# SparklingH/BloomScene

Measured on AMD Instinct MI355X. Metric: Msplats/s fwd+bwd @1M Gaussians 1920x1080 SH3; fraction of HBM roofline, higher is better.
Workload: dtype f32; 1 GPU; c3: 1000000 Gaussians, SH deg 3, 1920x1080, fwd+bwd colour+depth targets, synthetic scene A seed 0; gaussians=1000000, width=1920, height=1080, sh_degree=3, num_rendered=4386625, visible=1000000, parallelism=view-parallel x1, exact_exp=0, strict_gradients=0, prewarm_steps=292

## Files before the change

bloomscene_amd/csrc/api.hip:

```cpp
#include "../../include/bloomscene_rast.h"
#include "common.h"
#include "errors.h"
#include "host_state.h"
#include "launch.h"
#include "profiler.h"
#include "scratch.h"

#include <cstring>

using namespace bsr;

static constexpr unsigned BSR_KNOWN_FLAGS = BSR_FLAG_EXACT_EXP | BSR_FLAG_EXACT_GRAD | BSR_FLAG_NO_READBACK | BSR_FLAG_TEST_MASK;

static bool is_capturing(hipStream_t s)
{
	hipStreamCaptureStatus cs = hipStreamCaptureStatusNone;
	if (hipStreamIsCapturing(s, &cs) != hipSuccess) { (void)hipGetLastError(); cs = hipStreamCaptureStatusNone; }
	return cs != hipStreamCaptureStatusNone;
}

static int check_common(int P, int width, int height, const float* means3D, const float* scales, const float* rotations,
                        const float* cov3D_precomp, const float* viewmatrix, const float* projmatrix)
{
	if (P < 0 || width <= 0 || height <= 0) return fail("invalid sizes: P=%d width=%d height=%d", P, width, height);
// ... 139 lines not shown
	if (P_rows > 0x7fffffffu) return fail("too many (view, Gaussian) pairs for one call");

	char* geom_p = geometryBuffer(geometry_user, GeomState::bytes(P_rows));
	char* img_p = imageBuffer(image_user, ImgState::bytes(N, (size_t)T));
	if (!geom_p || !img_p) return fail("scratch allocation callback returned null");
	ForwardCall c = {s, flags, debug, no_readback, V, P, width, height, gx, gy, T, n_wg, P_rows,
	                 GeomState::carve(geom_p, P_rows), ImgState::carve(img_p, N, (size_t)T),
	                 binningBuffer, binning_user, background, out_color, out_depth, 0};
	const GeomState& geom = c.geom;
	const ImgState& img = c.img;

	if (prefiltered) HIP_TRY(hipMemsetAsync(img.flags, 0, sizeof(int), s));

	{
		PreArgs a;
		memset(&a, 0, sizeof(a));
		a.P = P; a.D = D; a.M = M;
		a.means3D = means3D; a.scales = scales; a.scale_modifier = scale_modifier; a.rotations = rotations;
		a.opacities = opacities; a.shs = shs; a.cov3D_precomp = cov3D_precomp; a.colors_precomp = colors_precomp;
		a.viewmatrix = viewmatrix; a.projmatrix = projmatrix; a.cam_pos = cam_pos;
		a.W = width; a.H = height; a.tan_fovx = tan_fovx; a.tan_fovy = tan_fovy;
		a.focal_y = height / (2.0f * tan_fovy);
		a.focal_x = width / (2.0f * tan_fovx);
		a.gx = gx; a.gy = gy; a.prefiltered = prefiltered; a.radii = radii; a.geom = geom;
		a.flags = img.flags;
		a.n_views = V;
		if (V > 1)
			HIP_TRY(hipMemsetAsync(geom.hist1, 0, BSR_RADIX_BINS_ * hist1_columns((size_t)n_wg) * sizeof(uint32_t), s));
		{
			StageTimer t("preprocess", s);
			launch_preprocess(a, false, s);
		}
		STAGE_CHECK("preprocess", debug, s);
	}
	SyncCache* sc = sync_cache();
	if (!sc) return 1;
	const bool capturing = no_readback && is_capturing(s);
	{
		StageTimer t("scan_wg", s);
		launch_scans(n_wg, geom.wg_kept, geom.wg_area, img.flags, geom.hist1, capturing ? nullptr : sc->pinned_dev, s);
	}
	STAGE_CHECK("scan_wg", debug, s);

	const CallShape shape{P, width, height, V};
	if (no_readback) {
		if (!capturing) {
			HIP_TRY(hipEventRecord(sc->deferred, s));
// ... 289 lines not shown

	if (R > 0) {
		{
			StageTimer t("render_bwd", s);
			RenderBwdArgs w;
			w.gx = gx; w.gy = gy; w.W = width; w.H = height;
			w.tile_range = img.tile_range; w.point_list = bin.point_list; w.rec = geom.rec; w.wg_base = geom.wg_kept;
			w.bg = background; w.final_T = img.final_T; w.n_contrib = img.n_contrib; w.dL_dpix = dL_dpix;
			w.out_depth = out_depth; w.dL_depths = out_depth ? dL_depths : nullptr;
			w.masks_flag = img.flags + 6; w.slab = slab;
			w.strict = (flags & BSR_FLAG_EXACT_GRAD) != 0; w.capacity = R;
			launch_render_bwd(w, s);
		}
		STAGE_CHECK("render_bwd", debug, s);
	}
	BwdArgs a;
	memset(&a, 0, sizeof(a));
	a.P = P; a.D = D; a.M = M;
	a.means3D = means3D; a.radii = radii; a.shs = shs; a.scales = scales; a.rotations = rotations;
	a.scale_modifier = scale_modifier; a.cov3D_precomp = cov3D_precomp; a.viewmatrix = viewmatrix;
	a.projmatrix = projmatrix; a.campos = campos; a.tan_fovx = tan_fovx; a.tan_fovy = tan_fovy;
	a.focal_y = height / (2.0f * tan_fovy);
	a.focal_x = width / (2.0f * tan_fovx);
	a.geom = geom;
	a.slab = slab; a.depth_grad = out_depth != nullptr;
	a.kept_ptr = img.flags + 2; a.capacity = R;
	a.dL_dmean2D = dL_dmean2D; a.dL_dconic = dL_dconic; a.dL_dopacity = dL_dopacity; a.dL_dcolor = dL_dcolor;
	a.dL_dmean3D = dL_dmean3D; a.dL_dcov3D = dL_dcov3D; a.dL_dsh = dL_dsh; a.dL_dscale = dL_dscale; a.dL_drot = dL_drot;
	{
		StageTimer t("preprocess_bwd", s);
		launch_preprocess_bwd(a, s);
	}
	STAGE_CHECK("preprocess_bwd", debug, s);
	return 0;
}

int bsr_backward(int P, int D, int M, int R, const float* background, int width, int height, const float* means3D,
                 const float* shs, const float* colors_precomp, const float* scales, float scale_modifier,
                 const float* rotations, const float* cov3D_precomp, const float* viewmatrix, const float* projmatrix,
                 const float* campos, float tan_fovx, float tan_fovy, const int* radii, char* geom_buffer,
                 char* binning_buffer, char* image_buffer, const float* dL_dpix, const float* dL_depths,
                 float* dL_dmean2D, float* dL_dconic, float* dL_dopacity, float* dL_dcolor, float* dL_dmean3D,
                 float* dL_dcov3D, float* dL_dsh, float* dL_dscale, float* dL_drot, int debug, void* stream)
{
	(void)dL_depths;
	return bsr_backward_ex(P, D, M, R, background, width, height, means3D, shs, colors_precomp, scales, scale_modifier,
	                       rotations, cov3D_precomp, viewmatrix, projmatrix, campos, tan_fovx, tan_fovy, radii, geom_buffer,
// ... 22 lines not shown
```

bloomscene_amd/csrc/common.h:

```cpp
#pragma once
#include <hip/hip_runtime.h>
#include <stdint.h>

#define BSR_TILE 16
#define BSR_BLOCK 256
#define BSR_NEAR 0.2f
#define BSR_PACK_MAX_SRC 8

namespace bsr {

struct Carver;
#define BSR_REC 4
struct GeomState {
	float4* rec;
	uint32_t* inst_offset;
	uint32_t* wg_kept;
	uint32_t* wg_area;
	uint32_t* hist1;
	uint64_t* kept_mask;
	ushort4* rect;
	uint8_t* clamped;
	float* depth;
	static GeomState layout(Carver& c, size_t P);
	static size_t bytes(size_t P);
	static GeomState carve(char* p, size_t P);
};
struct BinElem {
	uint32_t x;
	uint32_t y;
	uint32_t z;
};
typedef float bsr_f32x4 __attribute__((ext_vector_type(4)));
typedef float bsr_f32x2 __attribute__((ext_vector_type(2)));
typedef bsr_f32x4 bsr_f32x4_a4 __attribute__((aligned(4)));
typedef bsr_f32x2 bsr_f32x2_a4 __attribute__((aligned(4)));
__host__ __device__ __forceinline__ constexpr int slab_row_floats(bool depth_grad) { return depth_grad ? 10 : 9; }
#define BSR_SLAB_ROW_BYTES 40
#define BSR_SLAB_TAIL_BYTES 16
typedef uint32_t bsr_u32x3 __attribute__((ext_vector_type(3)));
typedef bsr_u32x3 bsr_u32x3_a4 __attribute__((aligned(4)));
__device__ __forceinline__ BinElem load_elem(const BinElem* p)
{
	const bsr_u32x3 v = *reinterpret_cast<const bsr_u32x3_a4*>(p);
	return BinElem{v.x, v.y, v.z};
}
__device__ __forceinline__ void store_elem(BinElem* p, const BinElem e)
{
	*reinterpret_cast<bsr_u32x3_a4*>(p) = bsr_u32x3{e.x, e.y, e.z};
}
// ... 44 lines not shown
	static size_t bytes(size_t N, size_t T);
	static ImgState carve(char* p, size_t N, size_t T);
};

struct PreArgs {
	int P, D, M;
	const float* means3D;
	const float* scales;
	float scale_modifier;
	const float* rotations;
	const float* opacities;
	const float* shs;
	const float* cov3D_precomp;
	const float* colors_precomp;
	const float* viewmatrix;
	const float* projmatrix;
	const float* cam_pos;
	int W, H;
	float tan_fovx, tan_fovy, focal_x, focal_y;
	int gx, gy;
	int prefiltered;
	int* radii;
	int n_views;
	GeomState geom;
	int* flags;
};

struct BwdArgs {
	int P, D, M;
	const float* means3D;
	const int* radii;
	const float* shs;
	const float* scales;
	const float* rotations;
	float scale_modifier;
	const float* cov3D_precomp;
	const float* viewmatrix;
	const float* projmatrix;
	const float* campos;
	float tan_fovx, tan_fovy, focal_x, focal_y;
	GeomState geom;
	const float4* slab;
	int depth_grad;
	const int* kept_ptr;
	int capacity;
	float* dL_dmean2D;
	float* dL_dconic;
	float* dL_dopacity;
	float* dL_dcolor;
	float* dL_dmean3D;
	float* dL_dcov3D;
	float* dL_dsh;
	float* dL_dscale;
	float* dL_drot;
};

int fail(const char* fmt, ...);

int read_u32_blocking(const uint32_t* dev, uint32_t* out, hipStream_t s);

static inline size_t align_up(size_t x, size_t a) { return (x + a - 1) & ~(a - 1); }

__device__ __forceinline__ float bsr_expf(float x)
{
	if (x != x) return x;
	if (x < -104.0f) return 0.0f;
	if (x > 88.72284f) return __builtin_inff();
	const float k = __builtin_rintf(x * 1.44269504088896341f);
	float r = __builtin_fmaf(-k, 0.693359375f, x);
	r = __builtin_fmaf(-k, -2.12194440e-4f, r);
	float p = 1.0f / 5040.0f;
	p = __builtin_fmaf(p, r, 1.0f / 720.0f);
	p = __builtin_fmaf(p, r, 1.0f / 120.0f);
	p = __builtin_fmaf(p, r, 1.0f / 24.0f);
	p = __builtin_fmaf(p, r, 1.0f / 6.0f);
	p = __builtin_fmaf(p, r, 0.5f);
	p = __builtin_fmaf(p, r, 1.0f);
// ... 125 lines not shown
```

bloomscene_amd/csrc/preprocess.hip:

```cpp
#include "common.h"
#include "sh.h"
#include "tile_common.h"
#include "launch.h"

namespace bsr {

struct Cov2DTerms {
	float t0[3], t1[3];
	float tx, ty, tz;
	float xmul, ymul;
};

__device__ __forceinline__ void cov2d_terms(const float3 mean, float focal_x, float focal_y, float tan_fovx,
                                            float tan_fovy, const float* __restrict__ vm, Cov2DTerms& o)
{
	float tx = vm[0] * mean.x + vm[4] * mean.y + vm[8] * mean.z + vm[12];
	float ty = vm[1] * mean.x + vm[5] * mean.y + vm[9] * mean.z + vm[13];
	const float tz = vm[2] * mean.x + vm[6] * mean.y + vm[10] * mean.z + vm[14];
	const float limx = 1.3f * tan_fovx;
	const float limy = 1.3f * tan_fovy;
	const float txtz = tx / tz;
	const float tytz = ty / tz;
	tx = fminf(limx, fmaxf(-limx, txtz)) * tz;
	ty = fminf(limy, fmaxf(-limy, tytz)) * tz;
// ... 18 lines not shown
	const float A10 = t.t0[0] * c[1] + t.t0[1] * c[3] + t.t0[2] * c[4];
	const float A20 = t.t0[0] * c[2] + t.t0[1] * c[4] + t.t0[2] * c[5];
	const float A01 = t.t1[0] * c[0] + t.t1[1] * c[1] + t.t1[2] * c[2];
	const float A11 = t.t1[0] * c[1] + t.t1[1] * c[3] + t.t1[2] * c[4];
	const float A21 = t.t1[0] * c[2] + t.t1[1] * c[4] + t.t1[2] * c[5];
	a = A00 * t.t0[0] + A10 * t.t0[1] + A20 * t.t0[2];
	b = A01 * t.t0[0] + A11 * t.t0[1] + A21 * t.t0[2];
	cc = A01 * t.t1[0] + A11 * t.t1[1] + A21 * t.t1[2];
	a += 0.3f;
	cc += 0.3f;
}

__device__ __forceinline__ float ndc2pix(float v, int S) { return (float)(((v + 1.0) * S - 1.0) * 0.5); }

__device__ __forceinline__ void get_rect(float px, float py, int max_radius, int gx, int gy, int* rmin, int* rmax)
{
	rmin[0] = min(gx, max(0, (int)((px - max_radius) / BSR_TILE)));
	rmin[1] = min(gy, max(0, (int)((py - max_radius) / BSR_TILE)));
	rmax[0] = min(gx, max(0, (int)((px + max_radius + BSR_TILE - 1) / BSR_TILE)));
	rmax[1] = min(gy, max(0, (int)((py + max_radius + BSR_TILE - 1) / BSR_TILE)));
}


template <bool FILTER_ONLY, int COLOR = 0>
__global__ void __launch_bounds__(256) k_preprocess(const PreArgs a)
{
	const int idx = blockIdx.x * 256 + threadIdx.x;
	const bool in_range = idx < a.P;
	if (FILTER_ONLY && !in_range) return;
	const int view = (int)blockIdx.y;
	const int wg = view * (int)gridDim.x + (int)blockIdx.x;
	const int id = wg * 256 + (int)threadIdx.x;
	const int ty_off = view * a.gy;

	__shared__ uint32_t s_hist[256];
	if (!FILTER_ONLY) {
		s_hist[threadIdx.x] = 0;
		__syncthreads();
	}

	int radius_out = 0;
	ushort4 rect_out = make_ushort4(0, 0, 0, 0);
	uint64_t kept_mask = 0;
	float4 rq0 = make_float4(0.f, 0.f, 0.f, 0.f), rq1 = rq0, rq2 = rq0;

	const int ld = in_range ? idx : 0;
	float3 p = make_float3(a.means3D[3 * ld], a.means3D[3 * ld + 1], a.means3D[3 * ld + 2]);
	const float* vm = a.viewmatrix + 16 * view;
	const float* pm = a.projmatrix + 16 * view;
	float pvz = vm[2] * p.x + vm[6] * p.y + vm[10] * p.z + vm[14];
	const bool alive = in_range && !(pvz <= BSR_NEAR);
	if (in_range && !alive && a.prefiltered) a.flags[0] = 1;

	bool vis = false;
	float cov3D[6] = {0.f, 0.f, 0.f, 0.f, 0.f, 0.f};
	float conic_a = 0.f, conic_b = 0.f, conic_c = 0.f, pix_x = 0.f, pix_y = 0.f;
	int rmin[2] = {0, 0}, rmax[2] = {0, 0};
	if (alive) {
		const float hx = pm[0] * p.x + pm[4] * p.y + pm[8] * p.z + pm[12];
		const float hy = pm[1] * p.x + pm[5] * p.y + pm[9] * p.z + pm[13];
		const float hw = pm[3] * p.x + pm[7] * p.y + pm[11] * p.z + pm[15];
		const float p_w = 1.0f / (hw + 0.0000001f);
		const float projx = hx * p_w, projy = hy * p_w;

		if (a.cov3D_precomp != nullptr) {
#pragma unroll
			for (int k = 0; k < 6; k++) cov3D[k] = a.cov3D_precomp[(size_t)idx * 6 + k];
// ... 65 lines not shown
			if (vis) {
				li = (int)s_pack[0][t];
				p = make_float3(__uint_as_float(s_pack[1][t]), __uint_as_float(s_pack[2][t]), __uint_as_float(s_pack[3][t]));
#pragma unroll
				for (int k = 0; k < 6; k++) cov3D[k] = __uint_as_float(s_pack[4 + k][t]);
				conic_a = __uint_as_float(s_pack[10][t]); conic_b = __uint_as_float(s_pack[11][t]); conic_c = __uint_as_float(s_pack[12][t]);
				radius_out = (int)s_pack[13][t];
				pix_x = __uint_as_float(s_pack[14][t]); pix_y = __uint_as_float(s_pack[15][t]);
				rmin[0] = (int)s_pack[16][t]; rmin[1] = (int)s_pack[17][t];
				rmax[0] = (int)s_pack[18][t]; rmax[1] = (int)s_pack[19][t];
				pvz = __uint_as_float(s_pack[20][t]);
			}
		}
	}
	const int gi = (int)blockIdx.x * 256 + li;
	const int gid = wg * 256 + li;

	if (vis) {
		rect_out = make_ushort4((unsigned short)rmin[0], (unsigned short)(rmin[1] + ty_off),
		                        (unsigned short)rmax[0], (unsigned short)(rmax[1] + ty_off));
		float rgb[3];
		uint8_t clamp_bits = 0;
		if (COLOR == 1) {
			sh3_to_rgb_stream(p, a.cam_pos + 3 * view, a.shs + (size_t)gi * 48, rgb, clamp_bits);
		} else if (COLOR == 0 && a.colors_precomp == nullptr) {
			sh_to_rgb(a.D, a.M, p, a.cam_pos + 3 * view, a.shs + (size_t)gi * a.M * 3, rgb, clamp_bits);
		} else {
			rgb[0] = a.colors_precomp[3 * gi];
			rgb[1] = a.colors_precomp[3 * gi + 1];
			rgb[2] = a.colors_precomp[3 * gi + 2];
		}
		const float opacity = a.opacities[gi];
		const float power_cut = -logf(255.0f * opacity) - 1.0e-3f;
		rq0 = make_float4(pix_x, pix_y, -0.5f * conic_a, -conic_b);
		rq1 = make_float4(-0.5f * conic_c, power_cut, opacity, pvz);
		a.geom.clamped[gid] = clamp_bits;
		const uint32_t area = (uint32_t)(rmax[0] - rmin[0]) * (uint32_t)(rmax[1] - rmin[1]);
		const bool pd = (conic_a > 0.0f) && (conic_c > 0.0f) && (conic_a * conic_c - conic_b * conic_b > 0.0f);
		const float rb_c = -conic_b / conic_c, rb_a = -conic_b / conic_a;
		if (area <= 64u) {
			int x0 = rmin[0], x1 = rmax[0], y0 = rmin[1], y1 = rmax[1];
			const float tq = -(power_cut - (1.0e-3f + 1.0e-4f * fabsf(power_cut)));
			const float cdet = conic_a * conic_c - conic_b * conic_b;
			if (pd) {
				if (tq < 0.0f) {
					x1 = x0;
				} else {
					const float hx = sqrtf(2.0f * tq * conic_c / cdet) * 1.0001f + 0.01f;
					const float hy = sqrtf(2.0f * tq * conic_a / cdet) * 1.0001f + 0.01f;
// ... 43 lines not shown
			const int per = ((int)(gridDim.x * gridDim.y) + 7) >> 3;
			if (a.n_views <= 1 || s_hist[threadIdx.x] != 0u)
				a.geom.hist1[(size_t)threadIdx.x * (8 * per) + hist1_column(wg, per)] = s_hist[threadIdx.x];
		}
		if (threadIdx.x == 0) {
			a.geom.wg_kept[wg] = w0 + w1 + w2 + w3;
			a.geom.wg_area[wg] = s_area[0] + s_area[1] + s_area[2] + s_area[3];
		}
		if (vis) {
			const uint32_t off = (wave > 0 ? w0 : 0u) + (wave > 1 ? w1 : 0u) + (wave > 2 ? w2 : 0u) + incl - n_inst;
			a.geom.rect[gid] = rect_out;
			a.geom.depth[gid] = rq1.w;
			a.geom.inst_offset[gid] = off;
			a.geom.kept_mask[gid] = kept_mask;
			{
				float4* rec = a.geom.rec + (size_t)gid * BSR_REC;
				rec[0] = rq0;
				rec[1] = rq1;
				rec[2] = rq2;
				rec[3] = make_float4(
				    __uint_as_float(off), __uint_as_float((uint32_t)rect_out.x | ((uint32_t)rect_out.y << 16)),
				    __uint_as_float((uint32_t)(rect_out.z - rect_out.x) | ((uint32_t)(rect_out.w - rect_out.y) << 16)),
				    __uint_as_float((uint32_t)kept_mask));
			}
		}
	}
}

__global__ void __launch_bounds__(256) k_mark_visible(int P, const float* __restrict__ means3D,
                                                      const float* __restrict__ vm, uint8_t* __restrict__ present)
{
	const int idx = blockIdx.x * 256 + threadIdx.x;
	if (idx >= P) return;
	const float pvz = vm[2] * means3D[3 * idx] + vm[6] * means3D[3 * idx + 1] + vm[10] * means3D[3 * idx + 2] + vm[14];
	present[idx] = !(pvz <= BSR_NEAR);
}

struct FilterWaveLds {
	float g[9][64];
	uint32_t q[128];
	uint32_t seen[2][64];
};

__device__ __forceinline__ void filter_wave_sync()
{
	__builtin_amdgcn_fence(__ATOMIC_RELEASE, "wavefront");
// ... 166 lines not shown
}

void launch_visible_filter_views(int P, int V, const float* means3D, const float* scales, float scale_modifier,
                                 const float* rotations, const float* cov3D_precomp, const float* viewmatrices,
                                 const float* projmatrices, int W, int H, float tan_fovx, float tan_fovy, int* radii,
                                 const int* group_of_view, int n_groups, uint8_t* group_mask, uint32_t* wg_counts,
                                 uint32_t* group_counts, hipStream_t s)
{
	const int n_wg = (P + 255) / 256;
	hipLaunchKernelGGL(k_visible_filter_views, dim3(n_wg), dim3(256), 0, s, P, V, means3D, scales,
	                   scale_modifier, rotations, cov3D_precomp, viewmatrices, projmatrices, W, H,
	                   W / (2.0f * tan_fovx), H / (2.0f * tan_fovy), tan_fovx, tan_fovy, (W + BSR_TILE - 1) / BSR_TILE,
	                   (H + BSR_TILE - 1) / BSR_TILE, radii, group_of_view, n_groups, group_mask,
	                   group_counts != nullptr ? wg_counts : nullptr);
	if (group_counts != nullptr && n_groups > 0)
		hipLaunchKernelGGL(k_sum_group_counts, dim3(n_groups), dim3(256), 0, s, n_wg, wg_counts, group_counts);
}

void launch_preprocess(const PreArgs& a, bool filter_only, hipStream_t s)
{
	const int blocks = (a.P + 255) / 256;
	if (filter_only)
		hipLaunchKernelGGL((k_preprocess<true, 0>), dim3(blocks), dim3(256), 0, s, a);
	else if (a.colors_precomp == nullptr && a.D == 3 && a.M == 16)
		hipLaunchKernelGGL((k_preprocess<false, 1>), dim3(blocks, a.n_views > 1 ? a.n_views : 1), dim3(256), 0, s, a);
	else if (a.colors_precomp != nullptr)
		hipLaunchKernelGGL((k_preprocess<false, 2>), dim3(blocks, a.n_views > 1 ? a.n_views : 1), dim3(256), 0, s, a);
	else
		hipLaunchKernelGGL((k_preprocess<false, 0>), dim3(blocks, a.n_views > 1 ? a.n_views : 1), dim3(256), 0, s, a);
}

void launch_mark_visible(int P, const float* means3D, const float* vm, uint8_t* present, hipStream_t s)
{
	hipLaunchKernelGGL(k_mark_visible, dim3((P + 255) / 256), dim3(256), 0, s, P, means3D, vm, present);
}

}
```

bloomscene_amd/csrc/preprocess_bwd.hip:

```cpp
#include "common.h"
#include "sh.h"
#include "launch.h"

namespace bsr {


template <int N>
__device__ __forceinline__ void store_sh_grad(float* __restrict__ dst, int M, const float* v)
{
	const int total = M * 3;
	if ((M & 3) == 0) {
		float4* d4 = reinterpret_cast<float4*>(dst);
		constexpr int NV = (N + 3) / 4;
#pragma unroll
		for (int i = 0; i < NV; i++) {
			float4 o;
			o.x = (i * 4 + 0 < N) ? v[i * 4 + 0] : 0.f;
			o.y = (i * 4 + 1 < N) ? v[i * 4 + 1] : 0.f;
			o.z = (i * 4 + 2 < N) ? v[i * 4 + 2] : 0.f;
			o.w = (i * 4 + 3 < N) ? v[i * 4 + 3] : 0.f;
			if (i * 4 < total) d4[i] = o;
		}
		for (int i = NV; i < (total >> 2); i++) d4[i] = make_float4(0.f, 0.f, 0.f, 0.f);
	} else {
#pragma unroll
		for (int i = 0; i < N; i++)
			if (i < total) dst[i] = v[i];
		for (int i = N; i < total; i++) dst[i] = 0.f;
	}
}

__device__ __forceinline__ void zero_sh_grad(float* __restrict__ dst, int M)
{
	const int total = M * 3;
	if ((M & 3) == 0) {
		float4* d4 = reinterpret_cast<float4*>(dst);
		for (int i = 0; i < (total >> 2); i++) d4[i] = make_float4(0.f, 0.f, 0.f, 0.f);
	} else {
		for (int i = 0; i < total; i++) dst[i] = 0.f;
	}
}

template <int DEG>
__device__ __forceinline__ void sh_bwd_deg(const BwdArgs& a, int idx, const float3 m, const float* dcolor, float* dmean)
{
	constexpr int NC = (DEG + 1) * (DEG + 1);
	const float ox = m.x - a.campos[0], oy = m.y - a.campos[1], oz = m.z - a.campos[2];
	const float len = sqrtf((ox * ox + oy * oy) + oz * oz);
	const float x = ox / len, y = oy / len, z = oz / len;
	const uint8_t cl = a.geom.clamped[idx];
	float dL_dRGB[3] = {dcolor[0], dcolor[1], dcolor[2]};
	dL_dRGB[0] *= (cl & 1) ? 0.f : 1.f;
	dL_dRGB[1] *= (cl & 2) ? 0.f : 1.f;
	dL_dRGB[2] *= (cl & 4) ? 0.f : 1.f;
	{
		float dsh[NC * 3];
		sh_coef_grad<DEG>(x, y, z, dL_dRGB, dsh);
		store_sh_grad<NC * 3>(a.dL_dsh + (size_t)idx * a.M * 3, a.M, dsh);
	}
	__builtin_amdgcn_sched_barrier(0);
	float dL_ddir[3];
	{
		float c[NC * 3];
		load_sh<NC>(a.shs + (size_t)idx * a.M * 3, a.M, c);
		sh_dir_grad<DEG>(c, x, y, z, dL_dRGB, dL_ddir);
	}
	const float sum2 = ox * ox + oy * oy + oz * oz;
	const float invsum32 = 1.0f / sqrtf(sum2 * sum2 * sum2);
	dmean[0] += ((+sum2 - ox * ox) * dL_ddir[0] - oy * ox * dL_ddir[1] - oz * ox * dL_ddir[2]) * invsum32;
	dmean[1] += (-ox * oy * dL_ddir[0] + (sum2 - oy * oy) * dL_ddir[1] - oz * oy * dL_ddir[2]) * invsum32;
	dmean[2] += (-ox * oz * dL_ddir[0] - oy * oz * dL_ddir[1] + (sum2 - oz * oz) * dL_ddir[2]) * invsum32;
}

template <int DEG, int ROW_F4>
__device__ __forceinline__ void sh_bwd_coop_half(const BwdArgs& a, int idx, bool visible, const float3 m, const float* dcolor,
                                                 float* dmean, ShTile<ROW_F4, 32>& tile, int lane, int g0, int n_valid)
{
	constexpr int NC = (DEG + 1) * (DEG + 1);
	constexpr int N = NC * 3;
	constexpr int STRIDE = ShTile<ROW_F4, 32>::STRIDE;
	const float ox = m.x - a.campos[0], oy = m.y - a.campos[1], oz = m.z - a.campos[2];
	const float len = sqrtf((ox * ox + oy * oy) + oz * oz);
	const float x = visible ? ox / len : 0.f, y = visible ? oy / len : 0.f, z = visible ? oz / len : 0.f;
	const uint8_t cl = visible ? a.geom.clamped[idx] : (uint8_t)7;
	float dL_dRGB[3] = {0.f, 0.f, 0.f};
	if (visible) {
		dL_dRGB[0] = dcolor[0] * ((cl & 1) ? 0.f : 1.f);
		dL_dRGB[1] = dcolor[1] * ((cl & 2) ? 0.f : 1.f);
		dL_dRGB[2] = dcolor[2] * ((cl & 4) ? 0.f : 1.f);
	}
	const int half = lane >> 5;
	float4* const row = &tile.rows[(lane & 31) * STRIDE];
	{
		float b[NC];
		sh_coef_basis<DEG>(x, y, z, b);
#pragma unroll
		for (int h = 0; h < 2; h++) {
			if (half == h) {
#pragma unroll
				for (int i = 0; i < ROW_F4; i++) {
					float4 o;
					o.x = (i * 4 + 0 < N) ? b[(i * 4 + 0 < N) ? (i * 4 + 0) / 3 : 0] * dL_dRGB[(i * 4 + 0) % 3] : 0.f;
					o.y = (i * 4 + 1 < N) ? b[(i * 4 + 1 < N) ? (i * 4 + 1) / 3 : 0] * dL_dRGB[(i * 4 + 1) % 3] : 0.f;
					o.z = (i * 4 + 2 < N) ? b[(i * 4 + 2 < N) ? (i * 4 + 2) / 3 : 0] * dL_dRGB[(i * 4 + 2) % 3] : 0.f;
					o.w = (i * 4 + 3 < N) ? b[(i * 4 + 3 < N) ? (i * 4 + 3) / 3 : 0] * dL_dRGB[(i * 4 + 3) % 3] : 0.f;
					row[i] = o;
				}
			}
			__builtin_amdgcn_fence(__ATOMIC_RELEASE, "wavefront");
			__builtin_amdgcn_wave_barrier();
			__builtin_amdgcn_fence(__ATOMIC_ACQUIRE, "wavefront");
			sh_tile_store<ROW_F4, 32>(tile, a.dL_dsh, g0 + 32 * h, min(32, max(0, n_valid - 32 * h)), lane);
			__builtin_amdgcn_fence(__ATOMIC_RELEASE, "wavefront");
			__builtin_amdgcn_wave_barrier();
			__builtin_amdgcn_fence(__ATOMIC_ACQUIRE, "wavefront");
		}
	}
	const uint64_t vis_mask = __ballot(visible);
	if (vis_mask == 0ull) return;
	float dL_ddir[3] = {0.f, 0.f, 0.f};
#pragma unroll
	for (int h = 0; h < 2; h++) {
		if (((vis_mask >> (32 * h)) & 0xffffffffull) == 0ull) continue;
		sh_tile_load<ROW_F4, 32>(tile, a.shs, g0 + 32 * h, min(32, max(0, n_valid - 32 * h)), lane);
		__builtin_amdgcn_fence(__ATOMIC_RELEASE, "wavefront");
		__builtin_amdgcn_wave_barrier();
		__builtin_amdgcn_fence(__ATOMIC_ACQUIRE, "wavefront");
		if (visible && half == h) {
			const float* const c = reinterpret_cast<const float*>(row);
			float dx0, dy0, dz0, dx1, dy1, dz1, dx2, dy2, dz2;
			sh_dir_grad_channel<DEG, 0>(c, x, y, z, dx0, dy0, dz0);
			__builtin_amdgcn_sched_barrier(0);
			sh_dir_grad_channel<DEG, 1>(c, x, y, z, dx1, dy1, dz1);
			__builtin_amdgcn_sched_barrier(0);
			sh_dir_grad_channel<DEG, 2>(c, x, y, z, dx2, dy2, dz2);
			dL_ddir[0] = (dx0 * dL_dRGB[0] + dx1 * dL_dRGB[1]) + dx2 * dL_dRGB[2];
			dL_ddir[1] = (dy0 * dL_dRGB[0] + dy1 * dL_dRGB[1]) + dy2 * dL_dRGB[2];
			dL_ddir[2] = (dz0 * dL_dRGB[0] + dz1 * dL_dRGB[1]) + dz2 * dL_dRGB[2];
		}
		__builtin_amdgcn_fence(__ATOMIC_RELEASE, "wavefront");
		__builtin_amdgcn_wave_barrier();
		__builtin_amdgcn_fence(__ATOMIC_ACQUIRE, "wavefront");
	}
	if (visible) {
		const float sum2 = ox * ox + oy * oy + oz * oz;
		const float invsum32 = 1.0f / sqrtf(sum2 * sum2 * sum2);
		dmean[0] += ((+sum2 - ox * ox) * dL_ddir[0] - oy * ox * dL_ddir[1] - oz * ox * dL_ddir[2]) * invsum32;
		dmean[1] += (-ox * oy * dL_ddir[0] + (sum2 - oy * oy) * dL_ddir[1] - oz * oy * dL_ddir[2]) * invsum32;
		dmean[2] += (-ox * oz * dL_ddir[0] - oy * oz * dL_ddir[1] + (sum2 - oz * oz) * dL_ddir[2]) * invsum32;
	}
}

template <int ROW_F4>
__global__ void __launch_bounds__(256, (ROW_F4 == 12 ? 6 : 4)) k_preprocess_bwd(const BwdArgs a)
{
	const int idx = blockIdx.x * 256 + threadIdx.x;
	const bool in_range = idx < a.P;
	const bool overflow = __builtin_amdgcn_readfirstlane(*a.kept_ptr) > a.capacity;
	const ushort4 rc = (in_range && !overflow) ? a.geom.rect[idx] : make_ushort4(0, 0, 0, 0);
	const bool visible = in_range && !overflow && (a.radii ? (a.radii[idx] > 0) : (rc.z > rc.x && rc.w > rc.y));

	constexpr int STAGE_F4 = (ROW_F4 > 0 && 32 * (ROW_F4 + 1) > 192) ? 32 * (ROW_F4 + 1) : 192;
	__shared__ float4 s_stage[4][STAGE_F4];
	float g[9] = {0.f, 0.f, 0.f, 0.f, 0.f, 0.f, 0.f, 0.f, 0.f};
	float g_z = 0.f;
	{
// ... 261 lines not shown
```

bloomscene_amd/csrc/scratch.h:

```cpp
#pragma once
#include "common.h"

namespace bsr {

static constexpr size_t BSR_RADIX_BINS_ = 256;

struct Carver {
	char* base;
	size_t off = 0;
	template <class T> T* take(size_t n)
	{
		T* r = base ? (T*)(base + off) : nullptr;
		off += align_up(n * sizeof(T), 256);
		return r;
	}
};

static inline size_t hist1_columns(size_t n_wg) { return (n_wg + 7) / 8 * 8; }

inline GeomState GeomState::layout(Carver& c, size_t P)
{
	const size_t n_wg = (P + 255) / 256;
	GeomState g;
	g.rec = c.take<float4>(P * BSR_REC);
	g.inst_offset = c.take<uint32_t>(P);
	g.wg_kept = c.take<uint32_t>(n_wg);
	g.wg_area = c.take<uint32_t>(n_wg);
	g.hist1 = c.take<uint32_t>(BSR_RADIX_BINS_ * hist1_columns(n_wg) + 512);
	g.kept_mask = c.take<uint64_t>(P);
	g.rect = c.take<ushort4>(P);
	g.clamped = c.take<uint8_t>(P);
	g.depth = c.take<float>(P);
	return g;
}
inline size_t GeomState::bytes(size_t P) { Carver c{nullptr}; layout(c, P); return c.off + 256; }
inline GeomState GeomState::carve(char* p, size_t P) { Carver c{(char*)align_up((size_t)p, 256)}; return layout(c, P); }

inline BinState BinState::layout(Carver& c, size_t R, bool with_slab)
{
	BinState b;
	b.point_list = c.take<uint32_t>(R);
	Carver pingpong = c, slab = c;
	b.elems_a = pingpong.take<BinElem>(R);
	b.elems_b = pingpong.take<BinElem>(R);
	b.slab = (float4*)slab.take<char>(with_slab ? R * BSR_SLAB_ROW_BYTES + BSR_SLAB_TAIL_BYTES : 0);
	c.off = pingpong.off > slab.off ? pingpong.off : slab.off;
	b.hist = c.take<uint32_t>(BSR_RADIX_BINS_ * (BSR_HIST_BLOCKS_MAX + 1));
	return b;
}
inline size_t BinState::bytes(size_t R, bool with_slab) { Carver c{nullptr}; layout(c, R, with_slab); return c.off + 256; }
inline BinState BinState::carve(char* p, size_t R, bool with_slab) { Carver c{(char*)align_up((size_t)p, 256)}; return layout(c, R, with_slab); }

static inline bool backward_fits(size_t cap, size_t R, size_t kept)
{
	Carver c{nullptr};
// ... 20 lines not shown
```

bloomscene_amd/csrc/sh.h:

```cpp
#pragma once
#include "common.h"

namespace bsr {

__device__ static const float SH_C0 = 0.28209479177387814f;
__device__ static const float SH_C1 = 0.4886025119029199f;
__device__ static const float SH_C2[5] = {1.0925484305920792f, -1.0925484305920792f, 0.31539156525252005f,
                                          -1.0925484305920792f, 0.5462742152960396f};
__device__ static const float SH_C3[7] = {-0.5900435899266435f, 2.890611442640554f, -0.4570457994644658f,
                                          0.3731763325901154f,  -0.4570457994644658f, 1.445305721320277f,
                                          -0.5900435899266435f};

template <int NC>
__device__ __forceinline__ void load_sh(const float* __restrict__ sh, int M, float* c)
{
	if ((M & 3) == 0) {
		const float4* s4 = reinterpret_cast<const float4*>(sh);
		constexpr int NV = (NC * 3 + 3) / 4;
#pragma unroll
		for (int i = 0; i < NV; i++) {
			if (i * 4 < M * 3) {
				const float4 v = s4[i];
				if (i * 4 + 0 < NC * 3) c[i * 4 + 0] = v.x;
				if (i * 4 + 1 < NC * 3) c[i * 4 + 1] = v.y;
// ... 38 lines not shown
__device__ __forceinline__ float sh3_basis(int k, float x, float y, float z, float xx, float yy, float zz, float xy,
                                           float yz, float xz)
{
	switch (k) {
	case 0: return SH_C0;
	case 1: return SH_C1 * y;
	case 2: return SH_C1 * z;
	case 3: return SH_C1 * x;
	case 4: return SH_C2[0] * xy;
	case 5: return SH_C2[1] * yz;
	case 6: return SH_C2[2] * (2.0f * zz - xx - yy);
	case 7: return SH_C2[3] * xz;
	case 8: return SH_C2[4] * (xx - yy);
	case 9: return SH_C3[0] * y * (3.0f * xx - yy);
	case 10: return SH_C3[1] * xy * z;
	case 11: return SH_C3[2] * y * (4.0f * zz - xx - yy);
	case 12: return SH_C3[3] * z * (2.0f * zz - 3.0f * xx - 3.0f * yy);
	case 13: return SH_C3[4] * x * (4.0f * zz - xx - yy);
	case 14: return SH_C3[5] * z * (xx - yy);
	default: return SH_C3[6] * x * (xx - 3.0f * yy);
	}
}

__device__ __forceinline__ void sh_eval3_stream(const float* __restrict__ sh, float x, float y, float z, float* res)
{
	const float xx = x * x, yy = y * y, zz = z * z;
	const float xy = x * y, yz = y * z, xz = x * z;
	const float4* s4 = reinterpret_cast<const float4*>(sh);
	float r[3] = {0.f, 0.f, 0.f};
#ifndef BSR_SH_GROUP
#define BSR_SH_GROUP 6
#endif
	constexpr int GS = BSR_SH_GROUP;
	static_assert(12 % GS == 0, "twelve 16-byte loads");
#pragma unroll
	for (int g = 0; g < 12 / GS; g++) {
		if (g > 0) asm volatile("" : "+v"(s4), "+v"(r[0]), "+v"(r[1]), "+v"(r[2]));
		float v[4 * GS];
#pragma unroll
		for (int i = 0; i < GS; i++) {
			const float4 q = s4[GS * g + i];
			v[4 * i + 0] = q.x; v[4 * i + 1] = q.y; v[4 * i + 2] = q.z; v[4 * i + 3] = q.w;
		}
#pragma unroll
		for (int j = 0; j < 4 * GS; j++) {
			const int p = 4 * GS * g + j, k = p / 3, ch = p % 3;
			const float b = sh3_basis(k, x, y, z, xx, yy, zz, xy, yz, xz);
			if (k == 0) r[ch] = b * v[j];
			else if (k == 1 || k == 3) r[ch] = r[ch] - b * v[j];
			else r[ch] = r[ch] + b * v[j];
		}
	}
#pragma unroll
	for (int ch = 0; ch < 3; ch++) res[ch] = r[ch] + 0.5f;
}

__device__ __forceinline__ void sh_to_rgb(int deg, int M, const float3 pos, const float* __restrict__ campos,
                                          const float* __restrict__ sh, float* rgb, uint8_t& clamp_bits)
{
	float dx = pos.x - campos[0], dy = pos.y - campos[1], dz = pos.z - campos[2];
	const float len = sqrtf((dx * dx + dy * dy) + dz * dz);
	dx = dx / len; dy = dy / len; dz = dz / len;
	float raw[3];
	if (deg <= 0) {
		float c[3];
		load_sh<1>(sh, M, c);
		sh_eval<0>(c, dx, dy, dz, raw);
	} else if (deg == 1) {
		float c[12];
		load_sh<4>(sh, M, c);
		sh_eval<1>(c, dx, dy, dz, raw);
	} else if (deg == 2) {
		float c[27];
		load_sh<9>(sh, M, c);
		sh_eval<2>(c, dx, dy, dz, raw);
	} else {
		float c[48];
		load_sh<16>(sh, M, c);
		sh_eval<3>(c, dx, dy, dz, raw);
	}
	clamp_bits = 0;
#pragma unroll
	for (int ch = 0; ch < 3; ch++) {
		if (raw[ch] < 0) clamp_bits |= (uint8_t)(1u << ch);
		rgb[ch] = fmaxf(raw[ch], 0.0f);
	}
}

__device__ __forceinline__ void sh3_to_rgb_stream(const float3 pos, const float* __restrict__ campos,
                                                  const float* __restrict__ sh, float* rgb, uint8_t& clamp_bits)
{
	float dx = pos.x - campos[0], dy = pos.y - campos[1], dz = pos.z - campos[2];
	const float len = sqrtf((dx * dx + dy * dy) + dz * dz);
	dx = dx / len; dy = dy / len; dz = dz / len;
	float raw[3];
	sh_eval3_stream(sh, dx, dy, dz, raw);
	clamp_bits = 0;
#pragma unroll
	for (int ch = 0; ch < 3; ch++) {
		if (raw[ch] < 0) clamp_bits |= (uint8_t)(1u << ch);
		rgb[ch] = fmaxf(raw[ch], 0.0f);
	}
}

template <int DEG>
__device__ __forceinline__ void sh_coef_grad(float x, float y, float z, const float* dL_dRGB, float* dsh)
{
#define DSH(k, v)                                                    \
	do {                                                             \
		const float _v = (v);                                        \
		_Pragma("unroll") for (int ch = 0; ch < 3; ch++) dsh[(k) * 3 + ch] = _v * dL_dRGB[ch]; \
	} while (0)
	DSH(0, SH_C0);
	if (DEG > 0) {
		DSH(1, -SH_C1 * y);
		DSH(2, SH_C1 * z);
		DSH(3, -SH_C1 * x);
		if (DEG > 1) {
			const float xx = x * x, yy = y * y, zz = z * z;
// ... 106 lines not shown
			const float xx = x * x, yy = y * y, zz = z * z;
			const float xy = x * y, yz = y * z, xz = x * z;
			dRGBdx += SH_C2[0] * y * SH(4) + SH_C2[2] * 2.f * -x * SH(6) + SH_C2[3] * z * SH(7) + SH_C2[4] * 2.f * x * SH(8);
			dRGBdy += SH_C2[0] * x * SH(4) + SH_C2[1] * z * SH(5) + SH_C2[2] * 2.f * -y * SH(6) + SH_C2[4] * 2.f * -y * SH(8);
			dRGBdz += SH_C2[1] * y * SH(5) + SH_C2[2] * 2.f * 2.f * z * SH(6) + SH_C2[3] * x * SH(7);
			if (DEG > 2) {
				dRGBdx += (SH_C3[0] * SH(9) * 3.f * 2.f * xy + SH_C3[1] * SH(10) * yz +
				           SH_C3[2] * SH(11) * -2.f * xy + SH_C3[3] * SH(12) * -3.f * 2.f * xz +
				           SH_C3[4] * SH(13) * (-3.f * xx + 4.f * zz - yy) + SH_C3[5] * SH(14) * 2.f * xz +
				           SH_C3[6] * SH(15) * 3.f * (xx - yy));
				dRGBdy += (SH_C3[0] * SH(9) * 3.f * (xx - yy) + SH_C3[1] * SH(10) * xz +
				           SH_C3[2] * SH(11) * (-3.f * yy + 4.f * zz - xx) + SH_C3[3] * SH(12) * -3.f * 2.f * yz +
				           SH_C3[4] * SH(13) * -2.f * xy + SH_C3[5] * SH(14) * -2.f * yz +
				           SH_C3[6] * SH(15) * -3.f * 2.f * xy);
				dRGBdz += (SH_C3[1] * SH(10) * xy + SH_C3[2] * SH(11) * 4.f * 2.f * yz +
				           SH_C3[3] * SH(12) * 3.f * (2.f * zz - xx - yy) + SH_C3[4] * SH(13) * 4.f * 2.f * xz +
				           SH_C3[5] * SH(14) * (xx - yy));
			}
		}
	}
#undef SH
}

template <int ROW_F4, int ROWS = 64>
struct ShTile {
	static constexpr int STRIDE = ROW_F4 + 1;
	float4 rows[ROWS * STRIDE];
};

template <int ROW_F4, int ROWS>
__device__ __forceinline__ void sh_tile_load(ShTile<ROW_F4, ROWS>& t, const float* __restrict__ base, int g0, int n_valid,
                                             int lane)
{
	const float4* src = reinterpret_cast<const float4*>(base) + (size_t)g0 * ROW_F4;
	const int n_f4 = n_valid * ROW_F4;
#pragma unroll
	for (int i = 0; i < (ROW_F4 * ROWS + 63) / 64; i++) {
		const int n = i * 64 + lane;
		if (n < n_f4) {
			const int g = n / ROW_F4, part = n - g * ROW_F4;
			t.rows[g * ShTile<ROW_F4, ROWS>::STRIDE + part] = src[n];
		}
	}
}

template <int ROW_F4, int ROWS>
// ... 17 lines not shown
```

Baseline: 1054 Msplats/s.

## Cache SH direction Jacobian in forward to avoid rereading SH coefficients in backward

In single-view runs the forward preprocess now computes the 3x3 Jacobian of colour with respect to view direction while it evaluates SH, and stores it in a new structure-of-arrays buffer in geometry state. The backward preprocess loads these nine floats and takes a small dot product instead of rereading all 48 SH coefficients and recomputing the directional gradient. This trades SH reads and ALU work in backward for nine extra float writes per Gaussian in forward plus nine reads in backward. It also adds register pressure to the forward SH evaluation.

```diff
diff --git a/bloomscene_amd/csrc/api.hip b/bloomscene_amd/csrc/api.hip
--- a/bloomscene_amd/csrc/api.hip
+++ b/bloomscene_amd/csrc/api.hip
@@ -185,7 +185,7 @@
 		a.W = width; a.H = height; a.tan_fovx = tan_fovx; a.tan_fovy = tan_fovy;
 		a.focal_y = height / (2.0f * tan_fovy);
 		a.focal_x = width / (2.0f * tan_fovx);
-		a.gx = gx; a.gy = gy; a.prefiltered = prefiltered; a.radii = radii; a.geom = geom;
+		a.gx = gx; a.gy = gy; a.prefiltered = prefiltered; a.radii = radii; a.geom = geom; a.dir_jac = geom.dir_jac;
 		a.flags = img.flags;
 		a.n_views = V;
 		if (V > 1)
@@ -521,7 +521,7 @@
 	a.projmatrix = projmatrix; a.campos = campos; a.tan_fovx = tan_fovx; a.tan_fovy = tan_fovy;
 	a.focal_y = height / (2.0f * tan_fovy);
 	a.focal_x = width / (2.0f * tan_fovx);
-	a.geom = geom;
+	a.geom = geom; a.dir_jac = geom.dir_jac;
 	a.slab = slab; a.depth_grad = out_depth != nullptr;
 	a.kept_ptr = img.flags + 2; a.capacity = R;
 	a.dL_dmean2D = dL_dmean2D; a.dL_dconic = dL_dconic; a.dL_dopacity = dL_dopacity; a.dL_dcolor = dL_dcolor;
diff --git a/bloomscene_amd/csrc/common.h b/bloomscene_amd/csrc/common.h
--- a/bloomscene_amd/csrc/common.h
+++ b/bloomscene_amd/csrc/common.h
@@ -11,7 +11,7 @@
 
 struct Carver;
 #define BSR_REC 4
-struct GeomState {
+struct GeomCore {
 	float4* rec;
 	uint32_t* inst_offset;
 	uint32_t* wg_kept;
@@ -21,10 +21,14 @@
 	ushort4* rect;
 	uint8_t* clamped;
 	float* depth;
+};
+struct GeomState : GeomCore {
+	float* dir_jac;
 	static GeomState layout(Carver& c, size_t P);
 	static size_t bytes(size_t P);
 	static GeomState carve(char* p, size_t P);
 };
+__host__ __device__ __forceinline__ constexpr size_t dir_jac_stride(size_t P) { return (P + 63) & ~(size_t)63; }
 struct BinElem {
 	uint32_t x;
 	uint32_t y;
@@ -115,8 +119,9 @@
 	int prefiltered;
 	int* radii;
 	int n_views;
-	GeomState geom;
+	GeomCore geom;
 	int* flags;
+	float* dir_jac;
 };
 
 struct BwdArgs {
@@ -132,7 +137,7 @@
 	const float* projmatrix;
 	const float* campos;
 	float tan_fovx, tan_fovy, focal_x, focal_y;
-	GeomState geom;
+	GeomCore geom;
 	const float4* slab;
 	int depth_grad;
 	const int* kept_ptr;
@@ -146,6 +151,7 @@
 	float* dL_dsh;
 	float* dL_dscale;
 	float* dL_drot;
+	const float* dir_jac;
 };
 
 int fail(const char* fmt, ...);
diff --git a/bloomscene_amd/csrc/preprocess.hip b/bloomscene_amd/csrc/preprocess.hip
--- a/bloomscene_amd/csrc/preprocess.hip
+++ b/bloomscene_amd/csrc/preprocess.hip
@@ -64,8 +64,13 @@
 }
 
 
-template <bool FILTER_ONLY, int COLOR = 0>
-__global__ void __launch_bounds__(256) k_preprocess(const PreArgs a)
+#ifdef BSR_PRE_JAC_WAVES
+#define BSR_PRE_JAC_ATTR __attribute__((amdgpu_waves_per_eu(JAC && COLOR == 1 ? BSR_PRE_JAC_WAVES : 1)))
+#else
+#define BSR_PRE_JAC_ATTR
+#endif
+template <bool FILTER_ONLY, int COLOR = 0, bool JAC = false>
+__global__ void __launch_bounds__(256) BSR_PRE_JAC_ATTR k_preprocess(const PreArgs a)
 {
 	const int idx = blockIdx.x * 256 + threadIdx.x;
 	const bool in_range = idx < a.P;
@@ -85,6 +90,7 @@
 	ushort4 rect_out = make_ushort4(0, 0, 0, 0);
 	uint64_t kept_mask = 0;
 	float4 rq0 = make_float4(0.f, 0.f, 0.f, 0.f), rq1 = rq0, rq2 = rq0;
+	float jac[9] = {0.f, 0.f, 0.f, 0.f, 0.f, 0.f, 0.f, 0.f, 0.f};
 
 	const int ld = in_range ? idx : 0;
 	float3 p = make_float3(a.means3D[3 * ld], a.means3D[3 * ld + 1], a.means3D[3 * ld + 2]);
@@ -196,9 +202,9 @@
 		float rgb[3];
 		uint8_t clamp_bits = 0;
 		if (COLOR == 1) {
-			sh3_to_rgb_stream(p, a.cam_pos + 3 * view, a.shs + (size_t)gi * 48, rgb, clamp_bits);
+			sh3_to_rgb_stream<JAC>(p, a.cam_pos + 3 * view, a.shs + (size_t)gi * 48, rgb, clamp_bits, jac);
 		} else if (COLOR == 0 && a.colors_precomp == nullptr) {
-			sh_to_rgb(a.D, a.M, p, a.cam_pos + 3 * view, a.shs + (size_t)gi * a.M * 3, rgb, clamp_bits);
+			sh_to_rgb<JAC>(a.D, a.M, p, a.cam_pos + 3 * view, a.shs + (size_t)gi * a.M * 3, rgb, clamp_bits, jac);
 		} else {
 			rgb[0] = a.colors_precomp[3 * gi];
 			rgb[1] = a.colors_precomp[3 * gi + 1];
@@ -288,6 +294,12 @@
 				    __uint_as_float(off), __uint_as_float((uint32_t)rect_out.x | ((uint32_t)rect_out.y << 16)),
 				    __uint_as_float((uint32_t)(rect_out.z - rect_out.x) | ((uint32_t)(rect_out.w - rect_out.y) << 16)),
 				    __uint_as_float((uint32_t)kept_mask));
+			}
+			if (JAC) {
+				float* const j = a.dir_jac + gid;
+				const size_t js = dir_jac_stride((size_t)a.P);
+#pragma unroll
+				for (int k = 0; k < 9; k++) j[k * js] = jac[k];
 			}
 		}
 	}
@@ -500,12 +512,17 @@
 	const int blocks = (a.P + 255) / 256;
 	if (filter_only)
 		hipLaunchKernelGGL((k_preprocess<true, 0>), dim3(blocks), dim3(256), 0, s, a);
-	else if (a.colors_precomp == nullptr && a.D == 3 && a.M == 16)
-		hipLaunchKernelGGL((k_preprocess<false, 1>), dim3(blocks, a.n_views > 1 ? a.n_views : 1), dim3(256), 0, s, a);
 	else if (a.colors_precomp != nullptr)
 		hipLaunchKernelGGL((k_preprocess<false, 2>), dim3(blocks, a.n_views > 1 ? a.n_views : 1), dim3(256), 0, s, a);
+	else if (a.n_views > 1) {
+		if (a.D == 3 && a.M == 16)
+			hipLaunchKernelGGL((k_preprocess<false, 1, false>), dim3(blocks, a.n_views), dim3(256), 0, s, a);
+		else
+			hipLaunchKernelGGL((k_preprocess<false, 0, false>), dim3(blocks, a.n_views), dim3(256), 0, s, a);
+	} else if (a.D == 3 && a.M == 16)
+		hipLaunchKernelGGL((k_preprocess<false, 1, true>), dim3(blocks), dim3(256), 0, s, a);
 	else
-		hipLaunchKernelGGL((k_preprocess<false, 0>), dim3(blocks, a.n_views > 1 ? a.n_views : 1), dim3(256), 0, s, a);
+		hipLaunchKernelGGL((k_preprocess<false, 0, true>), dim3(blocks), dim3(256), 0, s, a);
 }
 
 void launch_mark_visible(int P, const float* means3D, const float* vm, uint8_t* present, hipStream_t s)
diff --git a/bloomscene_amd/csrc/preprocess_bwd.hip b/bloomscene_amd/csrc/preprocess_bwd.hip
--- a/bloomscene_amd/csrc/preprocess_bwd.hip
+++ b/bloomscene_amd/csrc/preprocess_bwd.hip
@@ -39,6 +39,20 @@
 	} else {
 		for (int i = 0; i < total; i++) dst[i] = 0.f;
 	}
+}
+
+__device__ __forceinline__ void load_dir_jac(const BwdArgs& a, int idx, float* j)
+{
+	const float* const p = a.dir_jac + idx;
+	const size_t js = dir_jac_stride((size_t)a.P);
+#pragma unroll
+	for (int k = 0; k < 9; k++) j[k] = p[k * js];
+}
+__device__ __forceinline__ void dir_jac_dot(const float* j, const float* dL_dRGB, float* dL_ddir)
+{
+	dL_ddir[0] = (j[0] * dL_dRGB[0] + j[1] * dL_dRGB[1]) + j[2] * dL_dRGB[2];
+	dL_ddir[1] = (j[3] * dL_dRGB[0] + j[4] * dL_dRGB[1]) + j[5] * dL_dRGB[2];
+	dL_ddir[2] = (j[6] * dL_dRGB[0] + j[7] * dL_dRGB[1]) + j[8] * dL_dRGB[2];
 }
 
 template <int DEG>
@@ -60,11 +74,19 @@
 	}
 	__builtin_amdgcn_sched_barrier(0);
 	float dL_ddir[3];
+#ifdef BSR_BWD_REREAD_SH
 	{
 		float c[NC * 3];
 		load_sh<NC>(a.shs + (size_t)idx * a.M * 3, a.M, c);
 		sh_dir_grad<DEG>(c, x, y, z, dL_dRGB, dL_ddir);
 	}
+#else
+	{
+		float j[9];
+		load_dir_jac(a, idx, j);
+		dir_jac_dot(j, dL_dRGB, dL_ddir);
+	}
+#endif
 	const float sum2 = ox * ox + oy * oy + oz * oz;
 	const float invsum32 = 1.0f / sqrtf(sum2 * sum2 * sum2);
 	dmean[0] += ((+sum2 - ox * ox) * dL_ddir[0] - oy * ox * dL_ddir[1] - oz * ox * dL_ddir[2]) * invsum32;
@@ -91,6 +113,10 @@
 	}
 	const int half = lane >> 5;
 	float4* const row = &tile.rows[(lane & 31) * STRIDE];
+#ifndef BSR_BWD_REREAD_SH
+	float jac[9] = {0.f, 0.f, 0.f, 0.f, 0.f, 0.f, 0.f, 0.f, 0.f};
+	if (visible) load_dir_jac(a, idx, jac);
+#endif
 	{
 		float b[NC];
 		sh_coef_basis<DEG>(x, y, z, b);
@@ -116,6 +142,7 @@
 			__builtin_amdgcn_fence(__ATOMIC_ACQUIRE, "wavefront");
 		}
 	}
+#ifdef BSR_BWD_REREAD_SH
 	const uint64_t vis_mask = __ballot(visible);
 	if (vis_mask == 0ull) return;
 	float dL_ddir[3] = {0.f, 0.f, 0.f};
@@ -142,6 +169,10 @@
 		__builtin_amdgcn_wave_barrier();
 		__builtin_amdgcn_fence(__ATOMIC_ACQUIRE, "wavefront");
 	}
+#else
+	float dL_ddir[3] = {0.f, 0.f, 0.f};
+	if (visible) dir_jac_dot(jac, dL_dRGB, dL_ddir);
+#endif
 	if (visible) {
 		const float sum2 = ox * ox + oy * oy + oz * oz;
 		const float invsum32 = 1.0f / sqrtf(sum2 * sum2 * sum2);
diff --git a/bloomscene_amd/csrc/scratch.h b/bloomscene_amd/csrc/scratch.h
--- a/bloomscene_amd/csrc/scratch.h
+++ b/bloomscene_amd/csrc/scratch.h
@@ -31,6 +31,7 @@
 	g.rect = c.take<ushort4>(P);
 	g.clamped = c.take<uint8_t>(P);
 	g.depth = c.take<float>(P);
+	g.dir_jac = c.take<float>(9 * dir_jac_stride(P));
 	return g;
 }
 inline size_t GeomState::bytes(size_t P) { Carver c{nullptr}; layout(c, P); return c.off + 256; }
diff --git a/bloomscene_amd/csrc/sh.h b/bloomscene_amd/csrc/sh.h
--- a/bloomscene_amd/csrc/sh.h
+++ b/bloomscene_amd/csrc/sh.h
@@ -84,7 +84,8 @@
 	}
 }
 
-__device__ __forceinline__ void sh_eval3_stream(const float* __restrict__ sh, float x, float y, float z, float* res)
+template <bool JAC>
+__device__ __forceinline__ void sh_eval3_stream(const float* __restrict__ sh, float x, float y, float z, float* res, float* jac)
 {
 	const float xx = x * x, yy = y * y, zz = z * z;
 	const float xy = x * y, yz = y * z, xz = x * z;
@@ -95,9 +96,17 @@
 #endif
 	constexpr int GS = BSR_SH_GROUP;
 	static_assert(12 % GS == 0, "twelve 16-byte loads");
+	static_assert(!JAC || GS == 6, "the Jacobian's sums are split for two groups of six");
+	float jx[3], jy[3], jz[3], px[3], py[3];
 #pragma unroll
 	for (int g = 0; g < 12 / GS; g++) {
-		if (g > 0) asm volatile("" : "+v"(s4), "+v"(r[0]), "+v"(r[1]), "+v"(r[2]));
+		if (g > 0) {
+			asm volatile("" : "+v"(s4), "+v"(r[0]), "+v"(r[1]), "+v"(r[2]));
+			if (JAC)
+				asm volatile("" : "+v"(jx[0]), "+v"(jx[1]), "+v"(jx[2]), "+v"(jy[0]), "+v"(jy[1]), "+v"(jy[2]), "+v"(jz[0]),
+				             "+v"(jz[1]), "+v"(jz[2]), "+v"(px[0]), "+v"(px[1]), "+v"(px[2]), "+v"(py[0]), "+v"(py[1]),
+				             "+v"(py[2]));
+		}
 		float v[4 * GS];
 #pragma unroll
 		for (int i = 0; i < GS; i++) {
@@ -112,13 +121,50 @@
 			else if (k == 1 || k == 3) r[ch] = r[ch] - b * v[j];
 			else r[ch] = r[ch] + b * v[j];
 		}
+		if (JAC) {
+#pragma unroll
+			for (int ch = 0; ch < 3; ch++) {
+#define SH(k) v[(k) * 3 + ch - 4 * GS * g]
+				if (g == 0) {
+					jx[ch] = -SH_C1 * SH(3);
+					jy[ch] = -SH_C1 * SH(1);
+					jz[ch] = SH_C1 * SH(2);
+					px[ch] = SH_C2[0] * y * SH(4) + SH_C2[2] * 2.f * -x * SH(6) + SH_C2[3] * z * SH(7);
+					py[ch] = SH_C2[0] * x * SH(4) + SH_C2[1] * z * SH(5) + SH_C2[2] * 2.f * -y * SH(6);
+					jz[ch] += SH_C2[1] * y * SH(5) + SH_C2[2] * 2.f * 2.f * z * SH(6) + SH_C2[3] * x * SH(7);
+				} else {
+					jx[ch] += px[ch] + SH_C2[4] * 2.f * x * SH(8);
+					jy[ch] += py[ch] + SH_C2[4] * 2.f * -y * SH(8);
+					jx[ch] += (SH_C3[0] * SH(9) * 3.f * 2.f * xy + SH_C3[1] * SH(10) * yz +
+					           SH_C3[2] * SH(11) * -2.f * xy + SH_C3[3] * SH(12) * -3.f * 2.f * xz +
+					           SH_C3[4] * SH(13) * (-3.f * xx + 4.f * zz - yy) + SH_C3[5] * SH(14) * 2.f * xz +
+					           SH_C3[6] * SH(15) * 3.f * (xx - yy));
+					jy[ch] += (SH_C3[0] * SH(9) * 3.f * (xx - yy) + SH_C3[1] * SH(10) * xz +
+					           SH_C3[2] * SH(11) * (-3.f * yy + 4.f * zz - xx) + SH_C3[3] * SH(12) * -3.f * 2.f * yz +
+					           SH_C3[4] * SH(13) * -2.f * xy + SH_C3[5] * SH(14) * -2.f * yz +
+					           SH_C3[6] * SH(15) * -3.f * 2.f * xy);
+					jz[ch] += (SH_C3[1] * SH(10) * xy + SH_C3[2] * SH(11) * 4.f * 2.f * yz +
+					           SH_C3[3] * SH(12) * 3.f * (2.f * zz - xx - yy) + SH_C3[4] * SH(13) * 4.f * 2.f * xz +
+					           SH_C3[5] * SH(14) * (xx - yy));
+				}
+#undef SH
+			}
+		}
 	}
 #pragma unroll
 	for (int ch = 0; ch < 3; ch++) res[ch] = r[ch] + 0.5f;
-}
-
+	if (JAC) {
+#pragma unroll
+		for (int ch = 0; ch < 3; ch++) { jac[ch] = jx[ch]; jac[3 + ch] = jy[ch]; jac[6 + ch] = jz[ch]; }
+	}
+}
+
+template <int DEG>
+__device__ __forceinline__ void sh_dir_jacobian(const float* c, float x, float y, float z, float* jac);
+
+template <bool JAC>
 __device__ __forceinline__ void sh_to_rgb(int deg, int M, const float3 pos, const float* __restrict__ campos,
-                                          const float* __restrict__ sh, float* rgb, uint8_t& clamp_bits)
+                                          const float* __restrict__ sh, float* rgb, uint8_t& clamp_bits, float* jac)
 {
 	float dx = pos.x - campos[0], dy = pos.y - campos[1], dz = pos.z - campos[2];
 	const float len = sqrtf((dx * dx + dy * dy) + dz * dz);
@@ -128,18 +174,22 @@
 		float c[3];
 		load_sh<1>(sh, M, c);
 		sh_eval<0>(c, dx, dy, dz, raw);
+		if (JAC) sh_dir_jacobian<0>(c, dx, dy, dz, jac);
 	} else if (deg == 1) {
 		float c[12];
 		load_sh<4>(sh, M, c);
 		sh_eval<1>(c, dx, dy, dz, raw);
+		if (JAC) sh_dir_jacobian<1>(c, dx, dy, dz, jac);
 	} else if (deg == 2) {
 		float c[27];
 		load_sh<9>(sh, M, c);
 		sh_eval<2>(c, dx, dy, dz, raw);
+		if (JAC) sh_dir_jacobian<2>(c, dx, dy, dz, jac);
 	} else {
 		float c[48];
 		load_sh<16>(sh, M, c);
 		sh_eval<3>(c, dx, dy, dz, raw);
+		if (JAC) sh_dir_jacobian<3>(c, dx, dy, dz, jac);
 	}
 	clamp_bits = 0;
 #pragma unroll
@@ -149,14 +199,15 @@
 	}
 }
 
+template <bool JAC>
 __device__ __forceinline__ void sh3_to_rgb_stream(const float3 pos, const float* __restrict__ campos,
-                                                  const float* __restrict__ sh, float* rgb, uint8_t& clamp_bits)
+                                                  const float* __restrict__ sh, float* rgb, uint8_t& clamp_bits, float* jac)
 {
 	float dx = pos.x - campos[0], dy = pos.y - campos[1], dz = pos.z - campos[2];
 	const float len = sqrtf((dx * dx + dy * dy) + dz * dz);
 	dx = dx / len; dy = dy / len; dz = dz / len;
 	float raw[3];
-	sh_eval3_stream(sh, dx, dy, dz, raw);
+	sh_eval3_stream<JAC>(sh, dx, dy, dz, raw, jac);
 	clamp_bits = 0;
 #pragma unroll
 	for (int ch = 0; ch < 3; ch++) {
@@ -309,6 +360,14 @@
 #undef SH
 }
 
+template <int DEG>
+__device__ __forceinline__ void sh_dir_jacobian(const float* c, float x, float y, float z, float* jac)
+{
+	sh_dir_grad_channel<DEG, 0>(c, x, y, z, jac[0], jac[3], jac[6]);
+	sh_dir_grad_channel<DEG, 1>(c, x, y, z, jac[1], jac[4], jac[7]);
+	sh_dir_grad_channel<DEG, 2>(c, x, y, z, jac[2], jac[5], jac[8]);
+}
+
 template <int ROW_F4, int ROWS = 64>
 struct ShTile {
 	static constexpr int STRIDE = ROW_F4 + 1;
```

Measured after the change: 1070 Msplats/s, median of 4. 1.02x the previous value.
